# Guenael/rtlsdr-ft8d

Measured on AMD Instinct MI355X. Metric: 15 s FT8 frames decoded/s, higher is better.
Workload: dtype f32; 1 GPU; configs[2]: batch of 4096 synthetic 15 s 3200 sps IQ frames per GPU, 20 CQ signals/frame SNR U[-18,0] dB, full pipeline incl. HIP LDPC(174,91) BP, K_MAX_CANDIDATES=120; frames_per_gpu=4096, global_frames=4096, parallelism=frame-sharded x1

## Files before the change

### rtlsdr_ft8d_amd/csrc/bp_math.h

```cpp
#pragma once
#include <hip/hip_runtime.h>

namespace bpm {

typedef float f2 __attribute__((ext_vector_type(2)));

__device__ __forceinline__ f2 pk_fma(f2 a, f2 b, f2 c) { return __builtin_elementwise_fma(a, b, c); }

__device__ __forceinline__ f2 rcp_pair(f2 b) {
    f2 r;
    r.x = __builtin_amdgcn_rcpf(b.x);
    r.y = __builtin_amdgcn_rcpf(b.y);
    return r;
}
__device__ __forceinline__ f2 div_pair_3(f2 a, f2 b) {
    const f2 r0 = rcp_pair(b);
    const f2 q0 = a * r0;
    const f2 e1 = pk_fma(-b, q0, a);
    return pk_fma(e1, r0, q0);
}
__device__ __forceinline__ f2 div_pair_5(f2 a, f2 b) {
    const f2 r0 = rcp_pair(b);
    const f2 one = { 1.0f, 1.0f };
    const f2 e0 = pk_fma(-b, r0, one);
    const f2 r1 = pk_fma(e0, r0, r0);
    const f2 q0 = a * r1;
    const f2 e1 = pk_fma(-b, q0, a);
    return pk_fma(e1, r1, q0);
}
__device__ __forceinline__ f2 div_pair_ieee(f2 a, f2 b) {
    f2 q;
    q.x = __fdiv_rn(a.x, b.x);
    q.y = __fdiv_rn(a.y, b.y);
    return q;
}
__device__ __forceinline__ float div_one_3(float a, float b) {
    const float r0 = __builtin_amdgcn_rcpf(b);
    const float q0 = a * r0;
    const float e1 = __builtin_fmaf(-b, q0, a);
    return __builtin_fmaf(e1, r0, q0);
}
__device__ __forceinline__ float div_one_5(float a, float b) {
    const float r0 = __builtin_amdgcn_rcpf(b);
    const float e0 = __builtin_fmaf(-b, r0, 1.0f);
    const float r1 = __builtin_fmaf(e0, r0, r0);
    const float q0 = a * r1;
    const float e1 = __builtin_fmaf(-b, q0, a);
    return __builtin_fmaf(e1, r1, q0);
}

__device__ __forceinline__ float clamp_497(float q, float x) {
    unsigned long long saved;
    asm("s_mov_b64 %1, exec\n\t"
        "v_cmpx_gt_f32_e64 vcc, |%2|, %3\n\t"
        "v_bfi_b32 %0, %4, 1.0, %2\n\t"
        "s_mov_b64 exec, %1"
        : "+v"(q), "=&s"(saved) : "v"(x), "s"(4.97f), "s"(0x7fffffffu) : "vcc");
    return q;
}
__device__ __forceinline__ f2 clamp_497(f2 q, f2 x) {
    unsigned long long saved;
    float q0 = q.x, q1 = q.y;
    asm("s_mov_b64 %2, exec\n\t"
        "v_cmpx_gt_f32_e64 vcc, |%3|, %5\n\t"
        "v_bfi_b32 %0, %6, 1.0, %3\n\t"
        "s_mov_b64 exec, %2\n\t"
        "v_cmpx_gt_f32_e64 vcc, |%4|, %5\n\t"
        "v_bfi_b32 %1, %6, 1.0, %4\n\t"
        "s_mov_b64 exec, %2"
        : "+v"(q0), "+v"(q1), "=&s"(saved) : "v"(x.x), "v"(x.y), "s"(4.97f), "s"(0x7fffffffu) : "vcc");
    return f2{ q0, q1 };
}

template <bool FAST>
__device__ __forceinline__ f2 tanh_pair(f2 x) {
    const f2 x2 = x * x;
    const f2 a = x * (945.0f + x2 * (105.0f + x2));
    const f2 b = 945.0f + x2 * (420.0f + x2 * 15.0f);
    return clamp_497(FAST ? div_pair_5(a, b) : div_pair_ieee(a, b), x);
}
template <bool FAST>
__device__ __forceinline__ float tanh_one(float x) {
    const float x2 = x * x;
    const float a = x * (945.0f + x2 * (105.0f + x2));
    const float b = 945.0f + x2 * (420.0f + x2 * 15.0f);
    return clamp_497(FAST ? div_one_5(a, b) : __fdiv_rn(a, b), x);
}

__device__ __forceinline__ float tanh_ref(float x) {
    if (x < -4.97f) return -1.0f;
    if (x > 4.97f) return 1.0f;
    const float x2 = x * x;
    const float a = x * (945.0f + x2 * (105.0f + x2));
    const float b = 945.0f + x2 * (420.0f + x2 * 15.0f);
    return __fdiv_rn(a, b);
}

__device__ __forceinline__ float vgpr_m735() {
    float r;
    asm("v_mov_b32 %0, 0xc437c000" : "=v"(r));
    return r;
}
template <bool FAST>
__device__ __forceinline__ f2 atanh_pair(f2 x, float m735 = -735.0f) {
    const f2 x2 = x * x;
    const f2 inner = FAST ? pk_fma(x2, f2{ 64.0f, 64.0f }, f2{ m735, m735 }) : (-735.0f + x2 * 64.0f);
    const f2 a = x * (945.0f + x2 * inner);
    const f2 b = (945.0f + x2 * (-1050.0f + x2 * 225.0f));
    return FAST ? div_pair_3(a, b) : div_pair_ieee(a, b);
}
template <bool FAST>
__device__ __forceinline__ float atanh_one(float x) {
    const float x2 = x * x;
    const float inner = FAST ? __builtin_fmaf(x2, 64.0f, -735.0f) : (-735.0f + x2 * 64.0f);
    const float a = x * (945.0f + x2 * inner);
    const float b = (945.0f + x2 * (-1050.0f + x2 * 225.0f));
    return FAST ? div_one_3(a, b) : __fdiv_rn(a, b);
}

__device__ __forceinline__ float llr_norm_factor(float variance) { return __builtin_sqrtf(__fdiv_rn(24.0f, variance)); }

constexpr float kTanhMinAbs = 0x1p-82f;
constexpr float kAtanhMinAbs = 0x1p-59f;
constexpr float kAtanhMaxAbs = 1.05f;

}
```

### rtlsdr_ft8d_amd/csrc/decode.hip

```cpp
#include "ft8gpu_internal.h"
#include "ft8_tables.h"
#include "unpack_dev.h"
#include "bp_math.h"
#include "ldpc_lds_layout.h"
#include <stddef.h>
#include <stdlib.h>
#include <type_traits>

namespace {

using bpm::f2;
using bpm::tanh_pair;
using bpm::tanh_one;
using bpm::atanh_pair;
using bpm::atanh_one;

constexpr int kMaxCheckGroups = 4;

struct DecodeTables {
    uint16_t edge_slot[3][64][3];
    uint64_t rowmask[2][64][3];
    uint8_t  row_valid[2][64];
    uint8_t  own6[64], own7[64];
    uint64_t group_mask[kMaxCheckGroups + 1][kMaxCheckGroups][3];
    uint16_t crc_bit[77];
};

__device__ DecodeTables d_tab;
__constant__ uint8_t c_gray[8] = { 0, 1, 3, 2, 5, 6, 4, 7 };

constexpr int kRows = 84;
constexpr int kTocFloats = kRows * 8;
constexpr int kWaveLds = kTocFloats + 192;

__host__ __device__ constexpr int slot_index(int m, int pos) {
    return pos < 4 ? 4 * m + pos : 4 * kRows + 4 * m + (pos - 4);
}

__device__ __forceinline__ float min3_abs(float a, float b, float c) {
    float r;
    asm("v_min3_f32 %0, |%1|, |%2|, |%3|" : "=v"(r) : "v"(a), "v"(b), "v"(c));
    return r;
}
__device__ __forceinline__ float add_f32(float a, float b) {
    float r;
    asm("v_add_f32 %0, %1, %2" : "=v"(r) : "v"(a), "v"(b));
    return r;
}

__device__ __forceinline__ f2 mul_bcast_lo(f2 a, f2 b) {
    f2 r;
    asm("v_pk_mul_f32 %0, %1, %2 op_sel_hi:[1,0]" : "=v"(r) : "v"(a), "v"(b));
    return r;
}
__device__ __forceinline__ f2 mul_bcast_hi(f2 a, f2 b) {
    f2 r;
    asm("v_pk_mul_f32 %0, %1, %2 op_sel:[0,1]" : "=v"(r) : "v"(a), "v"(b));
    return r;
}

__device__ __forceinline__ float any_f32() {
    float r;
    asm volatile("" : "=v"(r));
    return r;
}

__device__ __forceinline__ uint32_t guard_key(float v) { return (__float_as_uint(v) << 1) - 1u; }
constexpr uint32_t kGuardMin = ((127u - 59u) << 24) - 1u;

__device__ __forceinline__ void wave_lds_sync() {
    __builtin_amdgcn_fence(__ATOMIC_RELEASE, "wavefront");
    __builtin_amdgcn_wave_barrier();
    __builtin_amdgcn_fence(__ATOMIC_ACQUIRE, "wavefront");
}

__device__ __forceinline__ int wave_sum(int v) {
    v += __builtin_amdgcn_update_dpp(0, v, 0xB1, 0xF, 0xF, true);
    v += __builtin_amdgcn_update_dpp(0, v, 0x4E, 0xF, 0xF, true);
    v += __builtin_amdgcn_update_dpp(0, v, 0x141, 0xF, 0xF, true);
    v += __builtin_amdgcn_update_dpp(0, v, 0x140, 0xF, 0xF, true);
    v += __builtin_amdgcn_update_dpp(0, v, 0x142, 0xA, 0xF, true);
    v += __builtin_amdgcn_update_dpp(0, v, 0x143, 0xC, 0xF, true);
    return __builtin_amdgcn_readlane(v, 63);
}

__device__ __forceinline__ uint32_t wave_xor(uint32_t x) {
    int v = (int)x;
    v ^= __builtin_amdgcn_update_dpp(0, v, 0xB1, 0xF, 0xF, true);
    v ^= __builtin_amdgcn_update_dpp(0, v, 0x4E, 0xF, 0xF, true);
    v ^= __builtin_amdgcn_update_dpp(0, v, 0x141, 0xF, 0xF, true);
    v ^= __builtin_amdgcn_update_dpp(0, v, 0x140, 0xF, 0xF, true);
    v ^= __builtin_amdgcn_update_dpp(0, v, 0x142, 0xA, 0xF, true);
    v ^= __builtin_amdgcn_update_dpp(0, v, 0x143, 0xC, 0xF, true);
    return (uint32_t)__builtin_amdgcn_readlane(v, 63);
}

__host__ __device__ inline uint32_t crc14_82(const uint8_t *msg) {
    uint32_t rem = 0;
    int idx_byte = 0;
    for (int bit = 0; bit < 82; ++bit) {
        if ((bit & 7) == 0) rem ^= (uint32_t)msg[idx_byte++] << 6;
        if (rem & 0x2000u) rem = ((rem << 1) ^ 0x2757u) & 0xFFFFu;
        else rem = (rem << 1) & 0xFFFFu;
    }
    return rem & 0x3FFFu;
}

template <bool COUNT_ERRORS, int kCheckGroups>
__global__ __launch_bounds__(256)
void ft8_decode_kernel(const uint8_t *__restrict__ mag, const ft8gpu_candidate *__restrict__ cands,
                       const int32_t *__restrict__ counts, ft8gpu_decode_status *__restrict__ status,
                       int nframes, int max_candidates, int max_iters, int force_ieee_div,
                       unsigned blocks_per_frame, unsigned bpf_magic) {
    __shared__ __attribute__((aligned(16))) float s_mem[4][kWaveLds];

    const int lane = threadIdx.x & 63;
    const int wave = __builtin_amdgcn_readfirstlane(threadIdx.x >> 6);
    const unsigned nb = gridDim.x, per = nb >> 3, main_blocks = per << 3;
    const unsigned vb = blockIdx.x < main_blocks ? (blockIdx.x & 7u) * per + (blockIdx.x >> 3) : blockIdx.x;
    const int frame = blocks_per_frame == 1u ? (int)vb : (int)__umulhi(vb, bpf_magic);
    const int ci = (int)(vb - (unsigned)frame * blocks_per_frame) * 4 + wave;
    if (frame >= nframes || ci >= max_candidates) return;
    if (ci >= counts[frame]) return;

    float *toc = s_mem[wave];
    float *llr = toc + kTocFloats;
    float4 *planeLO = reinterpret_cast<float4 *>(toc);
    float4 *planeHI = planeLO + kRows;

    const ft8gpu_candidate cand = cands[(size_t)frame * max_candidates + ci];

    if (lane < 58) {
        const int k = lane;
        const int sym = k + ((k < 29) ? 7 : 14);
        const int block = cand.time_offset + sym;
        int l0 = 0, l1 = 0, l2 = 0;
        if (block >= 0 && block < kNumBlocks) {
            const int index = ((cand.time_offset * 2 + cand.time_sub) * 2 + cand.freq_sub) * kNumBin + cand.freq_offset;
            const uint8_t *ps = mag + (size_t)frame * kMagArray + index + sym * kBlockStride;
            int s2[8];
#pragma unroll
            for (int j = 0; j < 8; ++j) s2[j] = ps[c_gray[j]];
            l0 = max(max(s2[4], s2[5]), max(s2[6], s2[7])) - max(max(s2[0], s2[1]), max(s2[2], s2[3]));
            l1 = max(max(s2[2], s2[3]), max(s2[6], s2[7])) - max(max(s2[0], s2[1]), max(s2[4], s2[5]));
            l2 = max(max(s2[1], s2[3]), max(s2[5], s2[7])) - max(max(s2[0], s2[2]), max(s2[4], s2[6]));
        }
        llr[3 * k + 0] = (float)l0;
        llr[3 * k + 1] = (float)l1;
        llr[3 * k + 2] = (float)l2;
    }
    wave_lds_sync();

    float cw[3];
    bool has[3];
    int isum = 0, isum2 = 0;
#pragma unroll
    for (int r = 0; r < 3; ++r) {
        const int n = lane + 64 * r;
        has[r] = n < kLdpcN;
        cw[r] = has[r] ? llr[n] : 0.0f;
        const int v = (int)cw[r];
        isum += v;
        isum2 += v * v;
    }
    const float sum = (float)wave_sum(isum);
    const float sum2 = (float)wave_sum(isum2);
    const float inv_n = 1.0f / 174;
    const float variance = (sum2 - (sum * sum * inv_n)) * inv_n;
    const float norm_factor = bpm::llr_norm_factor(variance);
#pragma unroll
    for (int r = 0; r < 3; ++r) cw[r] = has[r] ? cw[r] * norm_factor : 0.0f;

    int slot[9];
#pragma unroll
    for (int r = 0; r < 3; ++r)
#pragma unroll
        for (int e = 0; e < 3; ++e) slot[3 * r + e] = d_tab.edge_slot[r][lane][e];
    uint64_t gmask[kCheckGroups][3];
    if (!COUNT_ERRORS) {
#pragma unroll
        for (int g = 0; g < kCheckGroups; ++g)
#pragma unroll
            for (int w = 0; w < 3; ++w) gmask[g][w] = d_tab.group_mask[kCheckGroups][g][w];
    }
    uint64_t rmask[2][3];
    bool rvalid[2];
#pragma unroll
    for (int rr = 0; rr < 2; ++rr) {
        rvalid[rr] = d_tab.row_valid[rr][lane] != 0;
#pragma unroll
        for (int w = 0; w < 3; ++w) rmask[rr][w] = COUNT_ERRORS ? d_tab.rowmask[rr][lane][w] : 0ull;
    }

    const int row6 = d_tab.own6[lane], row7 = d_tab.own7[lane];
    const bool has6 = row6 != kRows - 1, has7 = row7 != kRows - 1;
    if (lane < 8) toc[slot_index(kRows - 1, lane)] = 1.0f;
    wave_lds_sync();

    float cwh[3];
#pragma unroll
    for (int r = 0; r < 3; ++r) cwh[r] = cw[r] * -0.5f;
    const f2 cwh01 = { cwh[0], cwh[1] };
    const uint64_t has2_mask = __ballot(has[2]);
    int min_errors = kLdpcM;
    uint64_t B0 = 0, B1 = 0, B2 = 0;
    int iter = 0;
    bool fast_ok = !force_ieee_div;
    f2 PA[3] = { { 0.0f, 0.0f }, { 0.0f, 0.0f }, { 0.0f, 0.0f } }, PB = { 0.0f, 0.0f };
    float pc = 0.0f;
    const float m735 = bpm::vgpr_m735();

    auto first_half = [&](auto fast_tag) -> bool {
        constexpr bool FAST = decltype(fast_tag)::value;
        f2 A[3], B;
        float c2;
        if (iter > 0) {
#pragma unroll
            for (int r = 0; r < 2; ++r) A[r] = atanh_pair<FAST>(PA[r], m735);
            B = atanh_pair<FAST>(PB, m735);
            A[2] = f2{ any_f32(), any_f32() };
            c2 = any_f32();
            if (has[2]) {
                A[2] = atanh_pair<FAST>(PA[2], m735);
                c2 = atanh_one<FAST>(pc);
            }
        } else {
#pragma unroll
            for (int r = 0; r < 3; ++r) A[r] = f2{ 0.0f, 0.0f };
            B = f2{ 0.0f, 0.0f };
            c2 = 0.0f;
        }
        f2 X[3], Y;
        float z;
        if (FAST) {
            const f2 u01 = cwh01 + B;
            const float u2 = cwh[2] + c2;
            X[0] = f2{ u01.x, u01.x } + A[0];
            X[1] = f2{ u01.y, u01.y } + A[1];
            X[2] = f2{ u2, u2 } + A[2];
            Y.x = add_f32(add_f32(cwh[0], A[0].y), A[0].x);
            Y.y = add_f32(add_f32(cwh[1], A[1].y), A[1].x);
            z = add_f32(add_f32(cwh[2], A[2].y), A[2].x);
            B0 = __ballot((X[0].y + A[0].x) < 0.0f);
            B1 = __ballot((X[1].y + A[1].x) < 0.0f);
            B2 = __ballot((X[2].y + A[2].x) < 0.0f) & has2_mask;
        } else {
            const float ah0[3] = { B.x, B.y, c2 };
            float x0[3];
            bool bit[3];
#pragma unroll
            for (int r = 0; r < 3; ++r) {
                const float v0 = -2 * ah0[r], v1 = -2 * A[r].y, v2 = -2 * A[r].x;
                const float u = cw[r] + v0;
                bit[r] = has[r] && (((u + v1) + v2) > 0.0f);
                x0[r] = ((cw[r] + v1) + v2) * -0.5f;
                X[r].x = (u + v2) * -0.5f;
                X[r].y = (u + v1) * -0.5f;
            }
            Y.x = x0[0];
            Y.y = x0[1];
            z = x0[2];
            B0 = __ballot(bit[0]);
            B1 = __ballot(bit[1]);
            B2 = __ballot(bit[2]);
        }
        if ((B0 | B1 | B2) == 0ull) return true;

        bool full_check = true;
        if (!COUNT_ERRORS) {
            uint32_t odd = 0;
#pragma unroll
            for (int g = 0; g < kCheckGroups; ++g)
                odd |= (uint32_t)__popcll((B0 & gmask[g][0]) ^ (B1 & gmask[g][1]) ^ (B2 & gmask[g][2]));
            full_check = (odd & 1u) == 0;
        }
        if (full_check) {
            int errors = 0;
#pragma unroll
            for (int rr = 0; rr < 2; ++rr) {
                const uint64_t m0 = COUNT_ERRORS ? rmask[rr][0] : d_tab.rowmask[rr][lane][0];
                const uint64_t m1 = COUNT_ERRORS ? rmask[rr][1] : d_tab.rowmask[rr][lane][1];
                const uint64_t m2 = COUNT_ERRORS ? rmask[rr][2] : d_tab.rowmask[rr][lane][2];
                const int par = (__popcll(B0 & m0) + __popcll(B1 & m1) + __popcll(B2 & m2)) & 1;
                errors += __popcll(__ballot(rvalid[rr] && par));
            }
            if (COUNT_ERRORS) {
                if (errors < min_errors) {
                    min_errors = errors;
                    if (errors == 0) return true;
                }
            } else if (errors == 0) {
                min_errors = 0;
                return true;
            }
        }
        if (iter + 1 >= max_iters) { iter = max_iters; return true; }

        f2 t[4];
#pragma unroll
        for (int r = 0; r < 2; ++r) t[r] = tanh_pair<FAST>(X[r]);
        t[3] = tanh_pair<FAST>(Y);
#pragma unroll
        for (int r = 0; r < 2; ++r) {
            toc[slot[3 * r + 1]] = t[r].x;
            toc[slot[3 * r + 2]] = t[r].y;
        }
        toc[slot[0]] = t[3].x;
        toc[slot[3]] = t[3].y;
        if (has[2]) {
            t[2] = tanh_pair<FAST>(X[2]);
            const float tz = tanh_one<FAST>(z);
            toc[slot[7]] = t[2].x;
            toc[slot[8]] = t[2].y;
            toc[slot[6]] = tz;
        }
        return false;
    };

    for (;; ++iter) {
        if (iter >= max_iters) break;
        const bool stop = fast_ok ? first_half(std::true_type{}) : first_half(std::false_type{});
        if (stop) break;
        wave_lds_sync();

        if (has6) {
            const float4 lo = planeLO[row6], hi = planeHI[row6];
            const float v0 = lo.x, v1 = lo.y, v2 = lo.z, v3 = lo.w, v4 = hi.x, v5 = hi.y;
            const f2 o01 = (mul_bcast_hi(f2{ v1, v0 } * v2, f2{ lo.z, lo.w }) * v4) * v5;
            const float p2 = v0 * v1;
            const float p3 = p2 * v2;
            const float p4 = p3 * v3;
            const f2 o23 = (f2{ p2 * v3, p3 } * v4) * v5;
            const float o4 = p4 * v5, o5 = p4 * v4;
            planeLO[row6] = make_float4(o01.x, o01.y, o23.x, o23.y);
            *reinterpret_cast<float2 *>(planeHI + row6) = make_float2(o4, o5);
        }
        if (has7) {
            const float4 lo = planeLO[row7], hi = planeHI[row7];
            const float v0 = lo.x, v1 = lo.y, v2 = lo.z, v3 = lo.w, v4 = hi.x, v5 = hi.y, v6 = hi.z;
            const f2 h23 = { hi.z, hi.w };
            const f2 o01 = mul_bcast_lo((mul_bcast_hi(f2{ v1, v0 } * v2, f2{ lo.z, lo.w }) * v4) * v5, h23);
            const float p2 = v0 * v1;
            const float p3 = p2 * v2;
            const float p4 = p3 * v3;
            const f2 p45 = f2{ v5, v4 } * p4;
            const float p5 = p45.y;
            const f2 o23 = mul_bcast_lo((f2{ p2 * v3, p3 } * v4) * v5, h23);
            const f2 o45 = mul_bcast_lo(p45, h23);
            const float o6 = p5 * v5;
            planeLO[row7] = make_float4(o01.x, o01.y, o23.x, o23.y);
            planeHI[row7] = make_float4(o45.x, o45.y, o6, 1.0f);
        }
        wave_lds_sync();

#pragma unroll
        for (int r = 0; r < 2; ++r) PA[r] = f2{ toc[slot[3 * r + 2]], toc[slot[3 * r + 1]] };
        PB = f2{ toc[slot[0]], toc[slot[3]] };
        PA[2] = f2{ toc[slot[8]], toc[slot[7]] };
        pc = toc[slot[6]];
        bool guard_ok = true;
        if (iter > 0) {
            float mabs = min3_abs(pc, PA[2].x, PA[2].y);
            mabs = min3_abs(mabs, PB.x, PB.y);
            mabs = min3_abs(mabs, PA[0].x, PA[0].y);
            mabs = min3_abs(mabs, PA[1].x, PA[1].y);
            guard_ok = __all(mabs >= 0x1p-59f);
            if (!guard_ok) {
                uint32_t gmin = min(guard_key(pc), min(guard_key(PA[2].x), guard_key(PA[2].y)));
                gmin = min(gmin, min(guard_key(PB.x), guard_key(PB.y)));
#pragma unroll
                for (int r = 0; r < 2; ++r) gmin = min(gmin, min(guard_key(PA[r].x), guard_key(PA[r].y)));
                guard_ok = __all(gmin >= kGuardMin);
            }
        }
        fast_ok = guard_ok && !force_ieee_div;
    }

    uint32_t crc_calc = 0;
    if (min_errors == 0) {
        uint32_t c = ((B0 >> lane) & 1ull) ? d_tab.crc_bit[lane] : 0u;
        if (lane < 13 && ((B1 >> lane) & 1ull)) c ^= d_tab.crc_bit[64 + lane];
        crc_calc = wave_xor(c);
    }
    static_assert(sizeof(ft8gpu_decode_status) == 48, "record is 12 dwords");
    static_assert(offsetof(ft8gpu_decode_status, a91) == 10 && offsetof(ft8gpu_decode_status, text) == 22, "record layout");
    uint32_t *rec32 = reinterpret_cast<uint32_t *>(llr);
    char *rec = reinterpret_cast<char *>(llr);
    const uint64_t w0 = __brevll(B0);
    const uint64_t w1 = __brevll(B1) & 0xFFFFFFE000000000ull;
    if (lane < 12) {
        const uint32_t hi0 = (uint32_t)(w0 >> 32), lo0 = (uint32_t)w0, hi1 = (uint32_t)(w1 >> 32);
        uint32_t v = 0;
        if (lane == 0) v = ((uint32_t)min_errors & 0xFFFFu) | ((uint32_t)iter << 16);
        else if (lane == 2) v = (__builtin_bswap32(hi0) & 0xFFFFu) << 16;
        else if (lane == 3) v = (__builtin_bswap32(hi0) >> 16) | (__builtin_bswap32(lo0) << 16);
        else if (lane == 4) v = (__builtin_bswap32(lo0) >> 16) | (__builtin_bswap32(hi1) << 16);
        else if (lane == 5) v = __builtin_bswap32(hi1) >> 16;
        rec32[lane] = v;
    }
    if (min_errors == 0) {
        const uint32_t crc_extracted = (uint32_t)(w1 >> 37) & 0x3FFFu;
        wave_lds_sync();
        if (lane == 0) {
            rec32[1] = crc_extracted | (crc_calc << 16);
            if (crc_extracted == crc_calc) {
                const int rc = ft8dev::unpack77(w0, w1 & 0xFFF8000000000000ull, rec + offsetof(ft8gpu_decode_status, text));
                if (rc < 0) {
                    rec32[5] &= 0xFFFFu;
                    for (int i = 6; i < 12; ++i) rec32[i] = 0;
                }
                rec[offsetof(ft8gpu_decode_status, unpack_status)] = (char)rc;
                rec[offsetof(ft8gpu_decode_status, ok)] = rc >= 0 ? 1 : 0;
                rec[offsetof(ft8gpu_decode_status, pad)] = 0;
            }
        }
    }
    wave_lds_sync();
    if (lane < 12)
        reinterpret_cast<uint32_t *>(status + (size_t)frame * max_candidates + ci)[lane] = rec32[lane];
}

}

hipError_t decode_tables_init(hipStream_t s) {
    static DecodeTables h;
    for (int r = 0; r < 3; ++r)
        for (int l = 0; l < 64; ++l) {
            const int n = l + 64 * r;
            for (int e = 0; e < 3; ++e) {
                if (n >= kLdpcN) { h.edge_slot[r][l][e] = (uint16_t)slot_index(kRows - 1, e); continue; }
                const int m = kFT8_Mn[n][e] - 1;
                int pos = -1;
                for (int j = 0; j < kFT8_Num_rows[m]; ++j)
                    if (kFT8_Nm[m][j] - 1 == n) pos = j;
                h.edge_slot[r][l][e] = (uint16_t)slot_index(kLdsRowPos[m], pos);
            }
        }
    for (int rr = 0; rr < 2; ++rr)
        for (int l = 0; l < 64; ++l) {
            const int m = l + 64 * rr;
            h.row_valid[rr][l] = m < kLdpcM;
            h.rowmask[rr][l][0] = h.rowmask[rr][l][1] = h.rowmask[rr][l][2] = 0;
            if (m >= kLdpcM) continue;
            for (int j = 0; j < kFT8_Num_rows[m]; ++j) {
                const int n = kFT8_Nm[m][j] - 1;
                h.rowmask[rr][l][n >> 6] |= 1ull << (n & 63);
            }
        }
    {
        int owned[kLdpcM] = { 0 }, used[kRows] = { 0 };
        for (int l = 0; l < 64; ++l) {
            h.own6[l] = h.own7[l] = (uint8_t)(kRows - 1);
            const int m6 = kOwn6Row[l], m7 = kOwn7Row[l];
            if (m6 != 255) { if (m6 >= kLdpcM || kFT8_Num_rows[m6] != 6) abort(); h.own6[l] = kLdsRowPos[m6]; ++owned[m6]; }
            if (m7 != 255) { if (m7 >= kLdpcM || kFT8_Num_rows[m7] != 7) abort(); h.own7[l] = kLdsRowPos[m7]; ++owned[m7]; }
        }
        for (int m = 0; m < kLdpcM; ++m) { if (owned[m] != 1 || kLdsRowPos[m] >= kRows - 1 || used[kLdsRowPos[m]]++) abort(); }
        if (kLdsRowPos[kRows - 1] != kRows - 1) abort();
        for (int r = 0; r < 3; ++r)
            for (int l = 0; l < 64; ++l)
                if (kVarOf[r][l] != (l + 64 * r < kLdpcN ? l + 64 * r : 255)) abort();
    }
    for (int G = 1; G <= kMaxCheckGroups; ++G) {
        for (int g = 0; g < kMaxCheckGroups; ++g)
            for (int w = 0; w < 3; ++w) h.group_mask[G][g][w] = 0;
        for (int m = 0; m < kLdpcM; ++m)
            for (int j = 0; j < kFT8_Num_rows[m]; ++j) {
                const int n = kFT8_Nm[m][j] - 1;
                h.group_mask[G][m % G][n >> 6] ^= 1ull << (n & 63);
            }
    }
    for (int i = 0; i < 77; ++i) {
        uint8_t m[12] = { 0 };
        m[i >> 3] = (uint8_t)(0x80u >> (i & 7));
        h.crc_bit[i] = (uint16_t)crc14_82(m);
    }
    return hipMemcpyToSymbolAsync(HIP_SYMBOL(d_tab), &h, sizeof(h), 0, hipMemcpyHostToDevice, s);
}

hipError_t launch_decode(const uint8_t *mag, const ft8gpu_candidate *cands, const int32_t *counts,
                         ft8gpu_decode_status *status, int nframes, int max_candidates, int ldpc_iters,
                         bool count_errors, int force_ieee_div, hipStream_t s) {
    if (nframes < 1) return hipSuccess;
    const unsigned bpf = (unsigned)(max_candidates + 3) / 4;
    const unsigned long long nblocks = (unsigned long long)nframes * bpf;
    if (nblocks * bpf >= (1ull << 32)) return hipErrorInvalidValue;
    const unsigned magic = bpf == 1u ? 0u : (unsigned)((1ull << 32) / bpf) + 1u;
    if (count_errors)
        hipLaunchKernelGGL((ft8_decode_kernel<true, 1>), dim3((unsigned)nblocks), dim3(256), 0, s,
                           mag, cands, counts, status, nframes, max_candidates, ldpc_iters, force_ieee_div, bpf, magic);
    else
        hipLaunchKernelGGL((ft8_decode_kernel<false, 3>), dim3((unsigned)nblocks), dim3(256), 0, s,
                           mag, cands, counts, status, nframes, max_candidates, ldpc_iters, force_ieee_div, bpf, magic);
    return hipGetLastError();
}
```

Measured before the change: 1.025 million frames/s.

## Micro-optimize LDPC decode prologue: byte-max LLRs, fast norm sqrt, wider edge slots

Replaces the eight per-byte gray-coded loads with two 32-bit loads and SDWA byte-max instructions to form the symbol LLRs, which are stored as ints in LDS. The norm factor now uses a reciprocal-based divide and a hardware sqrt with a one-ulp correction when the variance lies in a normal range, keeping the IEEE path as a fallback. It also widens the edge_slot table to 32-bit entries, simplifies the spare-row init index and cw masking, and rewrites the ballot comparisons to drop an add. These are several small instruction-count cuts in the per-candidate prologue. Rounding behaviour could differ slightly from the old code.

```diff
diff --git a/rtlsdr_ft8d_amd/csrc/bp_math.h b/rtlsdr_ft8d_amd/csrc/bp_math.h
--- a/rtlsdr_ft8d_amd/csrc/bp_math.h
+++ b/rtlsdr_ft8d_amd/csrc/bp_math.h
@@ -118,7 +118,19 @@
     return FAST ? div_one_3(a, b) : __fdiv_rn(a, b);
 }
 
-__device__ __forceinline__ float llr_norm_factor(float variance) { return __builtin_sqrtf(__fdiv_rn(24.0f, variance)); }
+constexpr uint32_t kNormFastMinBits = 0x35800000u, kNormFastMaxBits = 0x49800000u;
+__device__ __forceinline__ float llr_norm_factor(float variance) {
+    if (__float_as_uint(variance) - kNormFastMinBits <= kNormFastMaxBits - kNormFastMinBits) {
+        const float q = div_one_3(24.0f, variance);
+        const float s = __builtin_amdgcn_sqrtf(q);
+        const float sm = __uint_as_float(__float_as_uint(s) - 1u), sp = __uint_as_float(__float_as_uint(s) + 1u);
+        const float tm = __builtin_fmaf(-sm, s, q), tp = __builtin_fmaf(-sp, s, q);
+        float r = tm <= 0.0f ? sm : s;
+        r = tp > 0.0f ? sp : r;
+        return r;
+    }
+    return __builtin_sqrtf(__fdiv_rn(24.0f, variance));
+}
 
 constexpr float kTanhMinAbs = 0x1p-82f;
 constexpr float kAtanhMinAbs = 0x1p-59f;
diff --git a/rtlsdr_ft8d_amd/csrc/decode.hip b/rtlsdr_ft8d_amd/csrc/decode.hip
--- a/rtlsdr_ft8d_amd/csrc/decode.hip
+++ b/rtlsdr_ft8d_amd/csrc/decode.hip
@@ -18,7 +18,7 @@
 constexpr int kMaxCheckGroups = 4;
 
 struct DecodeTables {
-    uint16_t edge_slot[3][64][3];
+    uint32_t edge_slot[3][64][3];
     uint64_t rowmask[2][64][3];
     uint8_t  row_valid[2][64];
     uint8_t  own6[64], own7[64];
@@ -27,7 +27,6 @@
 };
 
 __device__ DecodeTables d_tab;
-__constant__ uint8_t c_gray[8] = { 0, 1, 3, 2, 5, 6, 4, 7 };
 
 constexpr int kRows = 84;
 constexpr int kTocFloats = kRows * 8;
@@ -56,6 +55,19 @@
 __device__ __forceinline__ f2 mul_bcast_hi(f2 a, f2 b) {
     f2 r;
     asm("v_pk_mul_f32 %0, %1, %2 op_sel:[0,1]" : "=v"(r) : "v"(a), "v"(b));
+    return r;
+}
+
+template <int SA, int SB>
+__device__ __forceinline__ int max_bytes(uint32_t a, uint32_t b) {
+    int r;
+#define FT8_MAX_BYTES(A, B) asm("v_max_u32_sdwa %0, %1, %2 dst_sel:DWORD dst_unused:UNUSED_PAD src0_sel:BYTE_" #A " src1_sel:BYTE_" #B : "=v"(r) : "v"(a), "v"(b))
+    if constexpr (SA == 0 && SB == 1) FT8_MAX_BYTES(0, 1);
+    else if constexpr (SA == 2 && SB == 3) FT8_MAX_BYTES(2, 3);
+    else if constexpr (SA == 0 && SB == 3) FT8_MAX_BYTES(0, 3);
+    else if constexpr (SA == 1 && SB == 2) FT8_MAX_BYTES(1, 2);
+    else static_assert(SA != SA, "add the pair of byte selects to the list");
+#undef FT8_MAX_BYTES
     return r;
 }
 
@@ -130,6 +142,7 @@
 
     const ft8gpu_candidate cand = cands[(size_t)frame * max_candidates + ci];
 
+    int *illr = reinterpret_cast<int *>(llr);
     if (lane < 58) {
         const int k = lane;
         const int sym = k + ((k < 29) ? 7 : 14);
@@ -138,16 +151,17 @@
         if (block >= 0 && block < kNumBlocks) {
             const int index = ((cand.time_offset * 2 + cand.time_sub) * 2 + cand.freq_sub) * kNumBin + cand.freq_offset;
             const uint8_t *ps = mag + (size_t)frame * kMagArray + index + sym * kBlockStride;
-            int s2[8];
-#pragma unroll
-            for (int j = 0; j < 8; ++j) s2[j] = ps[c_gray[j]];
-            l0 = max(max(s2[4], s2[5]), max(s2[6], s2[7])) - max(max(s2[0], s2[1]), max(s2[2], s2[3]));
-            l1 = max(max(s2[2], s2[3]), max(s2[6], s2[7])) - max(max(s2[0], s2[1]), max(s2[4], s2[5]));
-            l2 = max(max(s2[1], s2[3]), max(s2[5], s2[7])) - max(max(s2[0], s2[2]), max(s2[4], s2[6]));
-        }
-        llr[3 * k + 0] = (float)l0;
-        llr[3 * k + 1] = (float)l1;
-        llr[3 * k + 2] = (float)l2;
+            uint32_t w0, w1;
+            __builtin_memcpy(&w0, ps, 4);
+            __builtin_memcpy(&w1, ps + 4, 4);
+            const int m01 = max_bytes<0, 1>(w0, w0), m23 = max_bytes<2, 3>(w0, w0), m45 = max_bytes<0, 1>(w1, w1), m67 = max_bytes<2, 3>(w1, w1);
+            l0 = max(m45, m67) - max(m01, m23);
+            l1 = max(m23, max_bytes<0, 3>(w1, w1)) - max(m01, max_bytes<1, 2>(w1, w1));
+            l2 = max(max_bytes<1, 2>(w0, w0), m67) - max(max_bytes<0, 3>(w0, w0), m45);
+        }
+        illr[3 * k + 0] = l0;
+        illr[3 * k + 1] = l1;
+        illr[3 * k + 2] = l2;
     }
     wave_lds_sync();
 
@@ -158,8 +172,8 @@
     for (int r = 0; r < 3; ++r) {
         const int n = lane + 64 * r;
         has[r] = n < kLdpcN;
-        cw[r] = has[r] ? llr[n] : 0.0f;
-        const int v = (int)cw[r];
+        const int v = has[r] ? illr[n] : 0;
+        cw[r] = (float)v;
         isum += v;
         isum2 += v * v;
     }
@@ -169,7 +183,7 @@
     const float variance = (sum2 - (sum * sum * inv_n)) * inv_n;
     const float norm_factor = bpm::llr_norm_factor(variance);
 #pragma unroll
-    for (int r = 0; r < 3; ++r) cw[r] = has[r] ? cw[r] * norm_factor : 0.0f;
+    for (int r = 0; r < 3; ++r) cw[r] = cw[r] * norm_factor;
 
     int slot[9];
 #pragma unroll
@@ -194,7 +208,8 @@
 
     const int row6 = d_tab.own6[lane], row7 = d_tab.own7[lane];
     const bool has6 = row6 != kRows - 1, has7 = row7 != kRows - 1;
-    if (lane < 8) toc[slot_index(kRows - 1, lane)] = 1.0f;
+    static_assert(slot_index(kRows - 1, 3) + 1 + 4 * (kRows - 1) == slot_index(kRows - 1, 4), "the spare row's second half lies 4 * (kRows - 1) further on");
+    if (lane < 8) toc[4 * (kRows - 1) + lane + (lane >> 2) * (4 * (kRows - 1))] = 1.0f;
     wave_lds_sync();
 
     float cwh[3];
@@ -241,9 +256,9 @@
             Y.x = add_f32(add_f32(cwh[0], A[0].y), A[0].x);
             Y.y = add_f32(add_f32(cwh[1], A[1].y), A[1].x);
             z = add_f32(add_f32(cwh[2], A[2].y), A[2].x);
-            B0 = __ballot((X[0].y + A[0].x) < 0.0f);
-            B1 = __ballot((X[1].y + A[1].x) < 0.0f);
-            B2 = __ballot((X[2].y + A[2].x) < 0.0f) & has2_mask;
+            B0 = __ballot(X[0].y < -A[0].x);
+            B1 = __ballot(X[1].y < -A[1].x);
+            B2 = __ballot(X[2].y < -A[2].x) & has2_mask;
         } else {
             const float ah0[3] = { B.x, B.y, c2 };
             float x0[3];
@@ -252,7 +267,7 @@
             for (int r = 0; r < 3; ++r) {
                 const float v0 = -2 * ah0[r], v1 = -2 * A[r].y, v2 = -2 * A[r].x;
                 const float u = cw[r] + v0;
-                bit[r] = has[r] && (((u + v1) + v2) > 0.0f);
+                bit[r] = has[r] && ((u + v1) > -v2);
                 x0[r] = ((cw[r] + v1) + v2) * -0.5f;
                 X[r].x = (u + v2) * -0.5f;
                 X[r].y = (u + v1) * -0.5f;
@@ -428,12 +443,12 @@
         for (int l = 0; l < 64; ++l) {
             const int n = l + 64 * r;
             for (int e = 0; e < 3; ++e) {
-                if (n >= kLdpcN) { h.edge_slot[r][l][e] = (uint16_t)slot_index(kRows - 1, e); continue; }
+                if (n >= kLdpcN) { h.edge_slot[r][l][e] = (uint32_t)slot_index(kRows - 1, e); continue; }
                 const int m = kFT8_Mn[n][e] - 1;
                 int pos = -1;
                 for (int j = 0; j < kFT8_Num_rows[m]; ++j)
                     if (kFT8_Nm[m][j] - 1 == n) pos = j;
-                h.edge_slot[r][l][e] = (uint16_t)slot_index(kLdsRowPos[m], pos);
+                h.edge_slot[r][l][e] = (uint32_t)slot_index(kLdsRowPos[m], pos);
             }
         }
     for (int rr = 0; rr < 2; ++rr)
```

Measured after the change: 1.037 million frames/s (median of 6 runs). +1.2%, better.
